# prstrive/SCGaussian

Hardware: AMD Instinct MI355X
Metric: train_iters_per_sec (higher is better)
Workload: dtype f32; 1 GPU; S2: 200000 Gaussians, 1008x756, SH degree 3, fwd+bwd per view (BASELINE configs[1] shape: LLFF-fern 3-view training, 200 k Gaussians @ 1008x756); gaussians=200000, width=1008, height=756, sh_degree=3, visible=174771, views=3, parallelism=single, ranks_seen=1, launched_by=single process, grad_bucket_bytes=0, grad_bucket_bytes_per_view=0

## Files before the change

### scgaussian_amd/csrc/binning_tiles.hip

```cpp
#include "scg_common.h"
#include "tile_sort.h"
#include "tile_walk.h"

#include <mutex>

namespace scg {

constexpr int kTileBlocksSmall = 128;
constexpr int kTileBlocksLarge = 256;
constexpr int64_t kLargeFrame = 1ll << 20;
constexpr int kLargeScene = 100000;
constexpr int kSortSmallMax = 2048;
constexpr int kSortDenseMax = 4096;
constexpr int kSortMidMax = 8192;
constexpr int kVeryLong = 16384;
constexpr int kSort8Max = 4096;
constexpr int kSortBigLdsMax = 16384;
constexpr int kMaxDynLds = 152 * 1024;

template <class F>
__device__ __forceinline__ void visit_instances(const uint2* __restrict__ rects, int grid_x, uint32_t ga, uint32_t gb,
                                                F&& f) {
    const int lane = lane_id();
    for (uint32_t g0 = ga; g0 < gb; g0 += kWave) {
// ... 115 lines not shown
    return sum;
}

__device__ __forceinline__ uint32_t block_exclusive_256(uint32_t v, uint32_t* s_red, uint32_t& total) {
    const int lane = lane_id(), w = wave_id();
    uint32_t inc = v;
#pragma unroll
    for (int off = 1; off < kWave; off <<= 1) {
        const uint32_t n = (uint32_t)__shfl_up((int)inc, off, kWave);
        if (lane >= off) inc += n;
    }
    __syncthreads();
    if (lane == kWave - 1) s_red[w] = inc;
    __syncthreads();
    uint32_t before = 0;
    total = 0;
#pragma unroll
    for (int k = 0; k < kScatterWaves; ++k) {
        const uint32_t sk = s_red[k];
        if (k < w) before += sk;
        total += sk;
    }
    return before + inc - v;
}

__device__ __forceinline__ void publish_tile_starts(int x, int n_tiles, const uint32_t* __restrict__ tile_total,
                                                    const uint32_t* __restrict__ tile_part,
                                                    uint32_t* __restrict__ tile_start, uint2* __restrict__ ranges,
                                                    uint32_t capacity, uint32_t* __restrict__ class_counts,
                                                    uint32_t* __restrict__ mid_tiles, uint32_t* __restrict__ big_tiles,
                                                    uint32_t small_max, const uint32_t* __restrict__ len_hist,
                                                    const uint8_t* __restrict__ tile_class,
                                                    uint32_t* __restrict__ cost_out, const uint32_t* __restrict__ bcost_in,
                                                    uint8_t* q_class ,
                                                    uint32_t* __restrict__ nr_out) {
    __shared__ uint32_t s_red[kScatterWaves];
    __shared__ uint32_t s_first[kLenClasses];
    __shared__ uint32_t s_cnt[kLenClasses];
    const int per = (n_tiles + 7) >> 3;
    const int t0 = x * per, t1 = min(t0 + per, n_tiles);
    const int lane = lane_id();
    if (threadIdx.x < kLenClasses) {
        uint32_t before = 0;
        for (int k = (int)threadIdx.x + 1; k < kLenClasses; ++k) before += len_hist[x * kLenClasses + k];
        s_first[threadIdx.x] = before;
        s_cnt[threadIdx.x] = 0u;
    }
    uint32_t carry = totals_before(tile_total, tile_part, min(t0, n_tiles), s_red);
    uint32_t* order = reinterpret_cast<uint32_t*>(ranges) + 2 * (size_t)n_tiles;
    for (int k0 = t0; k0 < t1; k0 += kScatterThreads) {
        const int t = k0 + (int)threadIdx.x;
        const bool in = t < t1;
        const uint32_t cnt = in ? tile_total[t] : 0u;
        uint32_t total;
        const uint32_t run = carry + block_exclusive_256(cnt, s_red, total);
        carry += total;
        uint32_t len = 0;
        if (in) {
            tile_start[t] = run;
            const uint32_t lo = min(run, capacity), hi = min(run + cnt, capacity);
            ranges[t] = (hi > lo) ? make_uint2(lo, hi) : make_uint2(0u, 0u);
            len = hi - lo;
            if (t == n_tiles - 1) {
                tile_start[n_tiles] = run + cnt;
                if (nr_out) *nr_out = run + cnt;
            }
            if (cost_out) cost_out[t] = 0u;
            const int c = (int)tile_class[t];
            order[t0 + s_first[c] + atomicAdd(&s_cnt[c], 1u)] = (uint32_t)t;
        }
        const bool is_big = len > (uint32_t)kSortMidMax, is_mid = !is_big && len > small_max;
        const uint64_t m_mid = __ballot(is_mid), m_big = __ballot(is_big);
        const uint64_t m_split = __ballot(len > (uint32_t)kVeryLong);
        if (lane == 0 && m_split) atomicAdd(&class_counts[3], (uint32_t)__popcll(m_split));
        uint32_t base_mid = 0, base_big = 0;
        if (lane == 0) {
            if (m_mid) base_mid = atomicAdd(&class_counts[0], (uint32_t)__popcll(m_mid));
            if (m_big) base_big = atomicAdd(&class_counts[1], (uint32_t)__popcll(m_big));
        }
        base_mid = (uint32_t)__shfl((int)base_mid, 0, kWave);
        base_big = (uint32_t)__shfl((int)base_big, 0, kWave);
        const uint64_t below = (lane == 0) ? 0ull : (~0ull >> (kWave - lane));
        if (is_mid) mid_tiles[base_mid + (uint32_t)__popcll(m_mid & below)] = (uint32_t)t;
        if (is_big) big_tiles[base_big + (uint32_t)__popcll(m_big & below)] = (uint32_t)t;
    }
    for (int k = max(t0, t1) + (int)threadIdx.x; k < t0 + per; k += kScatterThreads) order[k] = (uint32_t)n_tiles;

    uint32_t* order_q = order + (size_t)tile_order_slots(n_tiles);
    const int slots8 = tile_order_slots(n_tiles) >> 3;
    const int nq = 4 * max(t1 - t0, 0);
    __syncthreads();
    if (!bcost_in) {
        for (int e = threadIdx.x; e < 4 * slots8; e += kScatterThreads) {
            const uint32_t t = order[t0 + (e >> 2)];
            order_q[4 * (size_t)t0 + e] = (t < (uint32_t)n_tiles) ? 4u * t + (uint32_t)(e & 3) : 4u * (uint32_t)n_tiles;
        }
        return;
    }
    auto qclass = [&](int e) {
        const uint32_t c = bcost_in[4 * (size_t)t0 + e];
        const int k = (int)(__float_as_uint((float)c) >> 19) - ((127 + 4) << 4);
        return max(0, min(kLenClasses - 1, k));
    };
    if (threadIdx.x < kLenClasses) s_cnt[threadIdx.x] = 0u;
    __syncthreads();
    for (int e = threadIdx.x; e < nq; e += kScatterThreads) {
        const int c = qclass(e);
        q_class[e] = (uint8_t)c;
        atomicAdd(&s_cnt[c], 1u);
    }
    __syncthreads();
    if (threadIdx.x < kLenClasses) {
        uint32_t before = 0;
        for (int k = (int)threadIdx.x + 1; k < kLenClasses; ++k) before += s_cnt[k];
        s_first[threadIdx.x] = before;
    }
    __syncthreads();
    if (threadIdx.x < kLenClasses) s_cnt[threadIdx.x] = 0u;
    __syncthreads();
    for (int e = threadIdx.x; e < nq; e += kScatterThreads) {
        const int c = (int)q_class[e];
        order_q[4 * (size_t)t0 + s_first[c] + atomicAdd(&s_cnt[c], 1u)] = 4u * (uint32_t)t0 + (uint32_t)e;
    }
    for (int e = nq + (int)threadIdx.x; e < 4 * slots8; e += kScatterThreads) order_q[4 * (size_t)t0 + e] = 4u * (uint32_t)n_tiles;
}

__device__ __forceinline__ void band_rows(int gy, int band, int& r0, int& r1) {
    r0 = (int)((int64_t)gy * band / kBands);
    r1 = (int)((int64_t)gy * (band + 1) / kBands);
}

__global__ __launch_bounds__(kScatterThreads) void tile_scatter_kernel(const uint2* __restrict__ rects, uint32_t P,
                                                                   int grid_x, int grid_y, int n_slices,
                                                                   const uint32_t* __restrict__ table,
                                                                   const uint32_t* __restrict__ tile_total,
                                                                   const uint32_t* __restrict__ tile_part,
                                                                   uint32_t* __restrict__ point_list,
                                                                   uint32_t capacity,
                                                                   uint32_t* __restrict__ tile_start,
                                                                   uint2* __restrict__ ranges,
                                                                   uint32_t* __restrict__ class_counts,
                                                                   uint32_t* __restrict__ mid_tiles,
                                                                   uint32_t* __restrict__ big_tiles, uint32_t small_max,
                                                                   const uint32_t* __restrict__ len_hist,
                                                                   const uint8_t* __restrict__ tile_class,
                                                                   uint32_t* __restrict__ cost_out, int block_slices,
                                                                   const uint32_t* __restrict__ bcost_in,
                                                                   uint32_t* __restrict__ nr_out) {
    extern __shared__ __attribute__((aligned(16))) unsigned char smem[];
    uint32_t* cursor = reinterpret_cast<uint32_t*>(smem);
    __shared__ uint2 s_qrect[kScatterWaves][kQueue];
    __shared__ uint32_t s_qid[kScatterWaves][kQueue];
    __shared__ uint32_t s_red[2 * kScatterWaves];
    const int n_tiles = grid_x * grid_y;
    if (blockIdx.x < kBands) {
        publish_tile_starts((int)blockIdx.x, n_tiles, tile_total, tile_part, tile_start, ranges, capacity, class_counts,
                            mid_tiles, big_tiles, small_max, len_hist, tile_class, cost_out, bcost_in,
                            smem ,
                            nr_out);
        return;
    }
#ifdef SCG_PROBE_TIMELINE
    uint32_t* tl = cost_out ? cost_out + n_tiles + ((size_t)blockIdx.x * kScatterWaves + wave_id()) * 8 : nullptr;
    const uint32_t tl0 = (uint32_t)wall_clock64();
    uint32_t tl_walk = 0, tl_nwalk = 0, tl_most = 0;
#endif
    const int wg = (int)blockIdx.x - kBands;
    const int band = wg & (kBands - 1), slice = wg >> 3;
    int r0, r1;
    band_rows(grid_y, band, r0, r1);
    const int t_lo = r0 * grid_x, nt = (r1 - r0) * grid_x;
    if (nt == 0) return;
    const int w = wave_id(), lane = lane_id();
    uint32_t sa, sb, dummy;
    if (block_slices) {
        block_slice(P, (uint32_t)n_slices, (uint32_t)slice, sa, sb);
        sa = min(sa * (uint32_t)kBlock, P);
        sb = min(sb * (uint32_t)kBlock, P);
    } else {
        wave_slice(P, (uint32_t)n_slices, (uint32_t)slice, 0u, sa, dummy);
        wave_slice(P, (uint32_t)n_slices, (uint32_t)slice, (uint32_t)kBinWaves - 1u, dummy, sb);
    }
    const uint32_t ga = sa + (uint32_t)((uint64_t)(sb - sa) * w / kScatterWaves);
    const uint32_t gb = sa + (uint32_t)((uint64_t)(sb - sa) * (w + 1) / kScatterWaves);
    constexpr int kAhead = 2;
    auto fetch = [&](uint32_t g) { return (g < gb) ? rects[g] : make_uint2(0u, 0u); };
    uint2 r_q[kAhead];
#pragma unroll
    for (int a = 0; a < kAhead; ++a) r_q[a] = fetch(ga + (uint32_t)(a * kWave + lane));
    const uint32_t* row = table + (size_t)slice * n_tiles + t_lo;
    constexpr int kRowRegs = 8;
    uint32_t row_pre[kRowRegs];
#pragma unroll
    for (int j = 0; j < kRowRegs; ++j) {
        const int k = j * kScatterThreads + (int)threadIdx.x;
        row_pre[j] = (k < nt) ? row[k] : 0u;
    }
    {
        const int full = t_lo / kColTiles;
        uint32_t before = 0;
        const int tail_k = full * kColTiles + (int)threadIdx.x;
        const uint32_t part0 = tile_part[min((int)threadIdx.x, max(full - 1, 0))];
        const uint32_t tail0 = tile_total[min(tail_k, n_tiles - 1)];
        uint32_t tot_pre[kRowRegs];
#pragma unroll
        for (int j = 0; j < kRowRegs; ++j) tot_pre[j] = tile_total[t_lo + min(j * kScatterThreads + (int)threadIdx.x, nt - 1)];
#pragma unroll
        for (int j = 0; j < kRowRegs; ++j) {
            const int k = j * kScatterThreads + (int)threadIdx.x;
            if (k < nt) cursor[k] = tot_pre[j];
        }
        for (int k = kRowRegs * kScatterThreads + (int)threadIdx.x; k < nt; k += kScatterThreads) cursor[k] = tile_total[t_lo + k];
        if ((int)threadIdx.x < full) before += part0;
        if (tail_k < t_lo) before += tail0;
        for (int k = (int)threadIdx.x + kScatterThreads; k < full; k += kScatterThreads) before += tile_part[k];
#pragma unroll
        for (int off = 32; off > 0; off >>= 1) before += (uint32_t)__shfl_xor((int)before, off, kWave);
        __syncthreads();
        const int share = (nt + kScatterThreads - 1) / kScatterThreads;
        const int k_a = min((int)threadIdx.x * share, nt), k_b = min(k_a + share, nt);
        uint32_t mine = 0;
        for (int k = k_a; k < k_b; ++k) mine += cursor[k];
        uint32_t inc = mine;
#pragma unroll
        for (int off = 1; off < kWave; off <<= 1) {
            const uint32_t n = (uint32_t)__shfl_up((int)inc, off, kWave);
            if (lane >= off) inc += n;
        }
        if (lane == kWave - 1) { s_red[w] = inc; s_red[kScatterWaves + w] = before; }
        __syncthreads();
        uint32_t start = inc - mine;
#pragma unroll
        for (int k = 0; k < kScatterWaves; ++k) start += s_red[kScatterWaves + k] + (k < w ? s_red[k] : 0u);
        for (int k = k_a; k < k_b; ++k) {
            const uint32_t cnt = cursor[k];
            cursor[k] = start;
            start += cnt;
        }
        __syncthreads();
#pragma unroll
        for (int j = 0; j < kRowRegs; ++j) {
            const int k = j * kScatterThreads + (int)threadIdx.x;
            if (k < nt) cursor[k] += row_pre[j];
        }
        for (int k = kRowRegs * kScatterThreads + (int)threadIdx.x; k < nt; k += kScatterThreads) cursor[k] += row[k];
        if (threadIdx.x < kWave) cursor[nt + threadIdx.x] = 0u;
    }
    __syncthreads();

#ifdef SCG_PROBE_TIMELINE
    const uint32_t tl1 = (uint32_t)wall_clock64();
#endif
    uint2* qrect = s_qrect[w];
    uint32_t* qid = s_qid[w];
    auto drop = [&](uint32_t tile, uint32_t id) {
        const uint32_t pos = atomicAdd(&cursor[tile - (uint32_t)t_lo], 1u);
        if (pos < capacity) point_list[pos] = id;
    };
    auto scatter_rects = [&](uint2 r, uint32_t g) {
#ifdef SCG_PROBE_TIMELINE
        const uint32_t tw0 = (uint32_t)wall_clock64();
#endif
        const uint32_t wd = r.y & 0xFFFFu, ht = r.y >> 16;
        const uint32_t cnt = wd * ht;
        const uint32_t dump = (uint32_t)nt + (uint32_t)lane;
        uint32_t small = (cnt <= kCoopThreshold) ? cnt : 0u;
        uint32_t x = 0, row_tile = (r.x >> 16) * (uint32_t)grid_x + (r.x & 0xFFFFu) - (uint32_t)t_lo;
        uint32_t most = small;
#pragma unroll
        for (int off = 32; off > 0; off >>= 1) most = max(most, (uint32_t)__shfl_xor((int)most, off, kWave));
        for (uint32_t k = 0; k < most; k += 4) {
            uint32_t slot[4], pos[4];
#pragma unroll
            for (int u = 0; u < 4; ++u) {
                slot[u] = (k + u < small) ? row_tile + x : dump;
                if (++x == wd) { x = 0; row_tile += (uint32_t)grid_x; }
            }
#pragma unroll
            for (int u = 0; u < 4; ++u) pos[u] = atomicAdd(&cursor[slot[u]], 1u);
#pragma unroll
            for (int u = 0; u < 4; ++u)
                if (k + u < small && pos[u] < capacity) point_list[pos[u]] = g;
        }
        walk_rects(cnt > kCoopThreshold ? r : make_uint2(0u, 0u), g, grid_x, drop);
#ifdef SCG_PROBE_TIMELINE
        tl_walk += (uint32_t)wall_clock64() - tw0; tl_nwalk += 1; tl_most += most;
#endif
    };
    int qn = 0;
    for (uint32_t g0 = ga; g0 < gb; g0 += kWave) {
        const uint32_t g = g0 + lane;
        const uint2 r = r_q[0];
#pragma unroll
        for (int a = 0; a + 1 < kAhead; ++a) r_q[a] = r_q[a + 1];
        r_q[kAhead - 1] = fetch(g + kAhead * kWave);
        const int y0 = max((int)(r.x >> 16), r0), y1 = min((int)(r.x >> 16) + (int)(r.y >> 16), r1);
        const bool touches = (r.y & 0xFFFFu) != 0u && y1 > y0;
        const uint64_t m = __ballot(touches);
        if (touches) {
            const int at = qn + (int)__builtin_amdgcn_mbcnt_hi((uint32_t)(m >> 32), __builtin_amdgcn_mbcnt_lo((uint32_t)m, 0u));
            qrect[at] = make_uint2((r.x & 0xFFFFu) | ((uint32_t)y0 << 16), (r.y & 0xFFFFu) | ((uint32_t)(y1 - y0) << 16));
            qid[at] = g;
        }
        qn += __popcll(m);
        __builtin_amdgcn_fence(__ATOMIC_ACQ_REL, "wavefront");
        __builtin_amdgcn_wave_barrier();
        if (qn >= kWave) {
            const uint2 qr = qrect[lane];
            const uint32_t qg = qid[lane];
            const uint2 mr = qrect[kWave + lane];
            const uint32_t mg = qid[kWave + lane];
            __builtin_amdgcn_fence(__ATOMIC_ACQ_REL, "wavefront");
            __builtin_amdgcn_wave_barrier();
            qn -= kWave;
            if (lane < qn) { qrect[lane] = mr; qid[lane] = mg; }
            __builtin_amdgcn_fence(__ATOMIC_ACQ_REL, "wavefront");
            __builtin_amdgcn_wave_barrier();
            scatter_rects(qr, qg);
        }
    }
    if (qn > 0) {
        uint2 qr = make_uint2(0u, 0u);
        uint32_t qg = 0;
        if (lane < qn) { qr = qrect[lane]; qg = qid[lane]; }
        scatter_rects(qr, qg);
    }
#ifdef SCG_PROBE_TIMELINE
    if (tl && lane == 0) {
        tl[0] = tl0; tl[1] = tl1; tl[2] = (uint32_t)wall_clock64(); tl[3] = tl_walk; tl[4] = tl_nwalk; tl[5] = tl_most;
        tl[6] = gb - ga; tl[7] = 0xC0FFEEu;
    }
#endif
}

__device__ __forceinline__ void sort_tile_in_lds(uint64_t* s_keys, const uint32_t* __restrict__ depth_keys,
                                                 uint32_t* __restrict__ list, int n) {
    for (int i = threadIdx.x; i < n; i += (int)blockDim.x) {
        const uint32_t id = list[i];
        s_keys[i] = ((uint64_t)depth_keys[id] << 32) | (uint64_t)id;
    }
    __syncthreads();
    bitonic_sort_asc(s_keys, n, false);
    __syncthreads();
    for (int i = threadIdx.x; i < n; i += (int)blockDim.x) list[i] = (uint32_t)s_keys[i];
}

template <int NW, int MAX_N>
__global__ __launch_bounds__(NW * kWave) void tile_sort_kernel(const uint2* __restrict__ ranges,
                                                               const uint32_t* __restrict__ depth_keys,
                                                               uint32_t* __restrict__ point_list, int id_bits) {
    __shared__ TileSortLds<NW, MAX_N> L;
    const uint2 r = ranges[blockIdx.x];
    const int n = (int)(r.y - r.x);
    if (n < 2 || n > MAX_N) return;
    sort_one_tile<NW, MAX_N, MAX_N>(L, r, depth_keys, point_list, id_bits);
}

constexpr int kRareThreads = 16 * kWave;
constexpr int kLongBuckets = 8192;

__device__ __forceinline__ void sort_big_tile(unsigned char* smem, const uint2 r, const uint32_t* __restrict__ depth_keys,
                                              uint32_t* __restrict__ point_list, uint64_t* __restrict__ spill,
                                              uint64_t* __restrict__ spill2) {
    const int n = (int)(r.y - r.x);
    uint32_t* list = point_list + r.x;
    uint64_t* keys = spill + r.x;
    if (!sort_long_list<kRareThreads, kLongBuckets>(smem, depth_keys, list, n, keys, spill2 + r.x)) {
        __syncthreads();
        if (n <= kSortBigLdsMax) {
            sort_tile_in_lds(reinterpret_cast<uint64_t*>(smem), depth_keys, list, n);
        } else {
            for (int i = threadIdx.x; i < n; i += kRareThreads) {
                const uint32_t id = list[i];
                keys[i] = ((uint64_t)depth_keys[id] << 32) | (uint64_t)id;
            }
            __syncthreads();
            bitonic_sort_asc(keys, n, true);
            __syncthreads();
            for (int i = threadIdx.x; i < n; i += kRareThreads) list[i] = (uint32_t)keys[i];
        }
    }
}

constexpr int kSegTarget = 1024;
constexpr int kSplitBatch = 16;
constexpr int kSegMaxPerTile = 8192;
static_assert(kSegTarget + kLongBucketMax <= kSort8Max, "a segment must fit the 8-wave sort");
static_assert(kLongBucketMax <= kSegTarget, "consecutive bucket starts must be at most a segment apart: no segment index is skipped");

__device__ __forceinline__ bool split_long_list(unsigned char* smem, const uint2 r, const uint32_t* __restrict__ depth_keys,
                                                uint32_t* __restrict__ point_list, uint64_t* __restrict__ A,
                                                uint32_t* __restrict__ seg_count, uint2* __restrict__ segments) {
    constexpr int T = kRareThreads, NW = T / kWave, PER = kLongBuckets / T;
    uint32_t* cnt = reinterpret_cast<uint32_t*>(smem);
    uint32_t* cur = cnt + kLongBuckets + 4;
    uint32_t* red = cur + kLongBuckets;
    uint32_t* pm = red + 2 * NW + 4;
    const int n = (int)(r.y - r.x);
    uint32_t* list = point_list + r.x;
    const int t = threadIdx.x, w = wave_id(), lane = lane_id();
    const int n_seg = (n + kSegTarget - 1) / kSegTarget;
    if (n_seg > kSegMaxPerTile) return false;
    uint32_t kmin, kmax;
    {
        const uint32_t key = depth_keys[list[(int)(((int64_t)t * n) / T)]];
        kmin = key; kmax = key;
    }
    for (int b = t; b < kLongBuckets; b += T) cnt[b] = 0u;
    for (int m = t; m <= n_seg; m += T) pm[m] = (uint32_t)n;
#pragma unroll
    for (int off = 32; off > 0; off >>= 1) {
        kmin = min(kmin, (uint32_t)__shfl_xor((int)kmin, off, kWave));
        kmax = max(kmax, (uint32_t)__shfl_xor((int)kmax, off, kWave));
    }
    if (lane == 0) { red[2 * w] = kmin; red[2 * w + 1] = kmax; }
    __syncthreads();
#pragma unroll
    for (int k = 0; k < NW; ++k) { kmin = min(kmin, red[2 * k]); kmax = max(kmax, red[2 * k + 1]); }
    const int sh = __builtin_clz((kmax - kmin) | 1u);
    auto bucket_of = [&](uint64_t comp) {
        const uint32_t key = (uint32_t)(comp >> 32);
        return __umulhi((min(max(key, kmin), kmax) - kmin) << sh, (uint32_t)kLongBuckets);
    };
    for (int i0 = t; i0 < n; i0 += kSplitBatch * T) {
        uint32_t id[kSplitBatch], key[kSplitBatch];
#pragma unroll
        for (int u = 0; u < kSplitBatch; ++u) id[u] = list[min(i0 + u * T, n - 1)];
#pragma unroll
        for (int u = 0; u < kSplitBatch; ++u) key[u] = depth_keys[id[u]];
#pragma unroll
        for (int u = 0; u < kSplitBatch; ++u) {
            if (i0 + u * T < n) {
                const uint64_t comp = ((uint64_t)key[u] << 32) | (uint64_t)id[u];
                A[i0 + u * T] = comp;
                atomicAdd(&cnt[bucket_of(comp)], 1u);
            }
        }
    }
    __syncthreads();
// ... 341 lines not shown
```

### scgaussian_amd/csrc/geometry.hip

```cpp
#include "scg_common.h"
#include "tile_walk.h"

#include <type_traits>

#pragma clang fp contract(off)

namespace scg {

__constant__ const float kC0 = 0.28209479177387814f;
__constant__ const float kC1 = 0.4886025119029199f;
__constant__ const float kC2[5] = {1.0925484305920792f, -1.0925484305920792f, 0.31539156525252005f,
                                   -1.0925484305920792f, 0.5462742152960396f};
__constant__ const float kC3[7] = {-0.5900435899266435f, 2.890611442640554f, -0.4570457994644658f,
                                   0.3731763325901154f, -0.4570457994644658f, 1.445305721320277f,
                                   -0.5900435899266435f};

struct Mat16 { float m[16]; };

__device__ __forceinline__ Mat16 load16(const float* __restrict__ p) {
    Mat16 r;
#pragma unroll
    for (int i = 0; i < 16; ++i) r.m[i] = p[i];
    return r;
}
// ... 314 lines not shown
        const float lam1 = mid + sqrtf(fmaxf(mid * mid - p.det, 0.1f));
        const float radius_f = ceilf(3.0f * sqrtf(lam1));
        const float ndc_x = p.hx * p.m_w;
        const float ndc_y = p.hy * p.m_w;
        px = ((ndc_x + 1.0f) * (float)f.W - 1.0f) * 0.5f;
        py = ((ndc_y + 1.0f) * (float)f.H - 1.0f) * 0.5f;
        int minx, miny, maxx, maxy;
        tile_rect(px, py, radius_f, f.gx, f.gy, minx, miny, maxx, maxy);
        const int tiles = (maxx - minx) * (maxy - miny);
        ok = tiles > 0;
        if (ok) {
            my_tiles = (uint32_t)tiles;
            radius_i = (int)fminf(fmaxf(radius_f, 0.0f), 2.0e9f);
            rect = make_uint2((uint32_t)minx | ((uint32_t)miny << 16),
                              (uint32_t)(maxx - minx) | ((uint32_t)(maxy - miny) << 16));
            tz = p.tz;
        }
    }
    constexpr bool has_colors = DEG < 0;
    constexpr int K = has_colors ? 1 : (DEG + 1) * (DEG + 1);
    float sh[(3 * K + 3) / 4 * 4];
#ifdef SCG_PROBE_TIMELINE
    { float pin = con_a; asm volatile("" : "+v"(pin)); }
    const uint32_t tp_math = (uint32_t)wall_clock64();
#endif
    if (!has_colors) src.template load_sh<K>(ok ? i : 0, sh);
    between(rect);
#ifdef SCG_PROBE_TIMELINE
    const uint32_t tp_between = (uint32_t)wall_clock64();
    asm volatile("" : "+v"(sh[0]), "+v"(sh[(3 * K + 3) / 4 * 4 - 1]));
    const uint32_t tp_sh = (uint32_t)wall_clock64();
    g_tp[0] += tp_math - g_tp[4]; g_tp[1] += tp_between - tp_math; g_tp[2] += tp_sh - tp_between; g_tp[4] = tp_sh;
#endif
    if (ok) {
        float rgb[3];
        if (has_colors) {
            rgb[0] = in.rgb[0]; rgb[1] = in.rgb[1]; rgb[2] = in.rgb[2];
        } else {
            float dx = in.x - f.campos[0], dy = in.y - f.campos[1], dz = in.z - f.campos[2];
            const float len = sqrtf(dx * dx + dy * dy + dz * dz);
            dx = dx / len; dy = dy / len; dz = dz / len;
            eval_sh<(DEG < 0 ? 0 : DEG)>(sh, dx, dy, dz, rgb);
#pragma unroll
            for (int c = 0; c < 3; ++c) {
                rgb[c] = rgb[c] + 0.5f;
                if (rgb[c] < 0.0f) { clamp_bits |= (uint8_t)(1u << c); rgb[c] = 0.0f; }
            }
        }
        sa = make_float4(px, py, con_a, con_b);
        const float opa = in.opacity;
        sb = make_float4(con_c, opa, 2.0f * logf(255.0f * opa) * 1.001f + 0.01f, -con_b / con_c);
        sc = make_float4(rgb[0], rgb[1], rgb[2], tz);
    }
    const int lane = lane_id();
    stage[3 * lane + 0] = sa;
    stage[3 * lane + 1] = sb;
    stage[3 * lane + 2] = sc;
    reinterpret_cast<uint4*>(stage + 3 * kWave)[lane] = make_uint4((uint32_t)radius_i, (uint32_t)clamp_bits, rect.x, rect.y);
    return my_tiles;
}

template <int DEG, class Src>
__device__ __forceinline__ void geometry_forward_body(
    const FrameDev& f, const Src& src, float4* __restrict__ splats,
    int32_t* __restrict__ radii, uint8_t* __restrict__ clamped, uint2* __restrict__ rects,
    uint32_t* __restrict__ depth_keys, uint32_t* __restrict__ block_sums) {
    __shared__ uint32_t s_wave_sum[kBlock / kWave];
    __shared__ float4 s_stage[(kBlock / kWave) * kStageVec];
    const int i = blockIdx.x * kBlock + threadIdx.x;
    const bool valid = i < f.P;
    const GeoIn in = src.template load<(DEG < 0)>(valid ? i : f.P - 1);
    const Mat16 V = load16(f.view);
    const Mat16 PM = load16(f.proj);
    float4* stage = s_stage + kStageVec * wave_id();
#ifdef SCG_PROBE_TIMELINE
    uint32_t tp_dummy[5] = {0u, 0u, 0u, 0u, 0u};
#endif
    const uint32_t my_tiles = geometry_forward_one<DEG>(f, V, PM, i, valid, in, src, stage,
                                                        [](uint2) {}
#ifdef SCG_PROBE_TIMELINE
                                                        , tp_dummy
#endif
                                                        );
    flush_stage(stage, i - lane_id(), f.P, splats, radii, clamped, rects, depth_keys);

    uint32_t s = my_tiles;
#pragma unroll
    for (int off = 32; off > 0; off >>= 1) s += __shfl_down(s, off, kWave);
    if (lane_id() == 0) s_wave_sum[wave_id()] = s;
    __syncthreads();
    if (threadIdx.x == 0) block_sums[blockIdx.x] = s_wave_sum[0] + s_wave_sum[1] + s_wave_sum[2] + s_wave_sum[3];
}

template <int DEG>
__global__ __launch_bounds__(kBlock) void geometry_forward_kernel(
    FrameDev f, const float* __restrict__ means3D, const float* __restrict__ opacities,
    const float* __restrict__ shs, const float* __restrict__ colors_precomp, const float* __restrict__ scales,
    const float* __restrict__ rotations, const float* __restrict__ cov3D_precomp, float4* __restrict__ splats,
    int32_t* __restrict__ radii, uint8_t* __restrict__ clamped, uint2* __restrict__ rects,
    uint32_t* __restrict__ depth_keys, uint32_t* __restrict__ block_sums, int sh_vec16) {
    const TensorSource src{means3D, opacities, shs, colors_precomp, scales, rotations, cov3D_precomp, f.M, sh_vec16};
    geometry_forward_body<DEG>(f, src, splats, radii, clamped, rects, depth_keys, block_sums);
}

template <int DEG>
__global__ __launch_bounds__(kBlock) void geometry_forward_model_kernel(
    FrameDev f, ScgModel model, float4* __restrict__ splats, int32_t* __restrict__ radii, uint8_t* __restrict__ clamped,
    uint2* __restrict__ rects, uint32_t* __restrict__ depth_keys, uint32_t* __restrict__ block_sums) {
    const ModelSource src{model};
    geometry_forward_body<DEG>(f, src, splats, radii, clamped, rects, depth_keys, block_sums);
}

__host__ __device__ __forceinline__ size_t geometry_hist_stage_offset(int n_tiles, int max_blocks) {
    return ((size_t)(n_tiles + max_blocks) * sizeof(uint32_t) + 15) & ~(size_t)15;
}
__host__ __device__ __forceinline__ size_t geometry_hist_lds_bytes(int n_tiles, int max_blocks) {
    return geometry_hist_stage_offset(n_tiles, max_blocks) + (size_t)(kBinThreads / kWave) * kStageVec * sizeof(float4);
}

template <int DEG, class Src>
__device__ __forceinline__ void geometry_hist_body(
    const FrameDev& f, const Src& src, float4* __restrict__ splats,
    int32_t* __restrict__ radii, uint8_t* __restrict__ clamped, uint2* __restrict__ rects,
    uint32_t* __restrict__ depth_keys, uint32_t* __restrict__ block_sums,
    uint32_t* __restrict__ table, uint32_t* __restrict__ class_counts, uint32_t* __restrict__ len_hist, int max_blocks) {
    extern __shared__ __attribute__((aligned(16))) unsigned char smem[];
    uint32_t* hist = reinterpret_cast<uint32_t*>(smem);
    const int n_tiles = f.gx * f.gy;
    uint32_t* s_blk = hist + n_tiles;
    float4* stage = reinterpret_cast<float4*>(smem + geometry_hist_stage_offset(n_tiles, max_blocks)) + kStageVec * wave_id();
    uint32_t blk_a, blk_b;
    block_slice((uint32_t)f.P, gridDim.x, blockIdx.x, blk_a, blk_b);
    const int lane = lane_id();
    uint32_t chunk = 4u * blk_a + (uint32_t)wave_id();
    auto fetch = [&](uint32_t c) {
        const int g = (int)(c * kWave) + lane;
        return src.template load<(DEG < 0)>(min(g, f.P - 1));
    };
    const Mat16 V = load16(f.view);
    const Mat16 PM = load16(f.proj);
    if (blockIdx.x == 0) {
        if (threadIdx.x < 4) class_counts[threadIdx.x] = 0u;
        len_hist[threadIdx.x] = 0u;
    }
    for (int t = threadIdx.x; t < n_tiles + max_blocks; t += kBinThreads) hist[t] = 0;
    uint32_t* next_chunk = s_blk + (max_blocks - 1);
    __syncthreads();
    if (threadIdx.x == 0) *next_chunk = 4u * blk_a + (uint32_t)kBinWaves;
    __syncthreads();
    int pending = -1;
#ifdef SCG_PROBE_TIMELINE
    uint32_t g_tp[5] = {0u, 0u, 0u, 0u, (uint32_t)wall_clock64()};
    const uint32_t tp_begin = g_tp[4];
    uint32_t tp_iters = 0;
#endif
    while (chunk < 4u * blk_b) {
        const int i = (int)(chunk * kWave) + lane;
        const GeoIn in = fetch(chunk);
        uint32_t grabbed = 0;
        if (lane == 0) grabbed = atomicAdd(next_chunk, 1u);
        const uint32_t my_tiles = geometry_forward_one<DEG>(
            f, V, PM, i, i < f.P, in, src, stage, [&](uint2 rect) {
                if (pending >= 0) flush_stage(stage, pending, f.P, splats, radii, clamped, rects, depth_keys);
                walk_rects(rect, (uint32_t)i, f.gx, [&](uint32_t tile, uint32_t) { atomicAdd(&hist[tile], 1u); });
            }
#ifdef SCG_PROBE_TIMELINE
            , g_tp
#endif
            );
#ifdef SCG_PROBE_TIMELINE
        { const uint32_t t = (uint32_t)wall_clock64(); g_tp[3] += t - g_tp[4]; g_tp[4] = t; ++tp_iters; }
#endif
        pending = i - lane;
        uint32_t s = my_tiles;
#pragma unroll
        for (int off = 32; off > 0; off >>= 1) s += __shfl_down(s, off, kWave);
        if (lane == 0 && s) atomicAdd(&s_blk[(chunk >> 2) - blk_a], s);
        chunk = (uint32_t)__builtin_amdgcn_readfirstlane((int)grabbed);
    }
    if (pending >= 0) flush_stage(stage, pending, f.P, splats, radii, clamped, rects, depth_keys);
#ifdef SCG_PROBE_TIMELINE
    const uint32_t tp_loop_end = (uint32_t)wall_clock64();
#endif
    __syncthreads();
#ifdef SCG_PROBE_TIMELINE
    if (f.cost_out && lane == 0) {
        uint32_t* tl = f.cost_out + n_tiles + 65792 + ((size_t)blockIdx.x * kBinWaves + wave_id()) * 8;
        tl[0] = tp_begin; tl[1] = g_tp[0]; tl[2] = g_tp[1]; tl[3] = g_tp[2]; tl[4] = g_tp[3]; tl[5] = tp_loop_end;
        tl[6] = (uint32_t)wall_clock64(); tl[7] = 0xC0FFEE00u | tp_iters;
    }
#endif
    uint32_t* row = table + (size_t)blockIdx.x * n_tiles;
    for (int t = threadIdx.x; t < n_tiles; t += kBinThreads) row[t] = hist[t];
    for (uint32_t k = threadIdx.x; k < blk_b - blk_a; k += kBinThreads) block_sums[blk_a + k] = s_blk[k];
}

template <int DEG>
__global__ __launch_bounds__(kBinThreads) void geometry_hist_kernel(
    FrameDev f, const float* __restrict__ means3D, const float* __restrict__ opacities,
    const float* __restrict__ shs, const float* __restrict__ colors_precomp, const float* __restrict__ scales,
    const float* __restrict__ rotations, const float* __restrict__ cov3D_precomp, float4* __restrict__ splats,
    int32_t* __restrict__ radii, uint8_t* __restrict__ clamped, uint2* __restrict__ rects,
    uint32_t* __restrict__ depth_keys, uint32_t* __restrict__ block_sums, int sh_vec16,
    uint32_t* __restrict__ table, uint32_t* __restrict__ class_counts, uint32_t* __restrict__ len_hist, int max_blocks) {
    const TensorSource src{means3D, opacities, shs, colors_precomp, scales, rotations, cov3D_precomp, f.M, sh_vec16};
    geometry_hist_body<DEG>(f, src, splats, radii, clamped, rects, depth_keys, block_sums, table, class_counts, len_hist, max_blocks);
}

template <int DEG>
__global__ __launch_bounds__(kBinThreads) void geometry_hist_model_kernel(
    FrameDev f, ScgModel model, float4* __restrict__ splats, int32_t* __restrict__ radii, uint8_t* __restrict__ clamped,
    uint2* __restrict__ rects, uint32_t* __restrict__ depth_keys, uint32_t* __restrict__ block_sums,
    uint32_t* __restrict__ table, uint32_t* __restrict__ class_counts, uint32_t* __restrict__ len_hist, int max_blocks) {
    const ModelSource src{model};
    geometry_hist_body<DEG>(f, src, splats, radii, clamped, rects, depth_keys, block_sums, table, class_counts, len_hist, max_blocks);
}

template <int DEG>
__device__ __forceinline__ void sh_basis_grads(float x, float y, float z, float* basis, float* bx, float* by, float* bz) {
    basis[0] = kC0; bx[0] = by[0] = bz[0] = 0.f;
    if (DEG > 0) {
        basis[1] = -kC1 * y; bx[1] = 0.f; by[1] = -kC1; bz[1] = 0.f;
        basis[2] = kC1 * z;  bx[2] = 0.f; by[2] = 0.f; bz[2] = kC1;
        basis[3] = -kC1 * x; bx[3] = -kC1; by[3] = 0.f; bz[3] = 0.f;
    }
    if (DEG > 1) {
        const float xx = x * x, yy = y * y, zz = z * z, xy = x * y, yz = y * z, xz = x * z;
        basis[4] = kC2[0] * xy;                    bx[4] = kC2[0] * y; by[4] = kC2[0] * x; bz[4] = 0.f;
        basis[5] = kC2[1] * yz;                    bx[5] = 0.f; by[5] = kC2[1] * z; bz[5] = kC2[1] * y;
        basis[6] = kC2[2] * (2.0f * zz - xx - yy); bx[6] = kC2[2] * -2.0f * x; by[6] = kC2[2] * -2.0f * y; bz[6] = kC2[2] * 4.0f * z;
        basis[7] = kC2[3] * xz;                    bx[7] = kC2[3] * z; by[7] = 0.f; bz[7] = kC2[3] * x;
        basis[8] = kC2[4] * (xx - yy);             bx[8] = kC2[4] * 2.0f * x; by[8] = kC2[4] * -2.0f * y; bz[8] = 0.f;
        if (DEG > 2) {
            basis[9] = kC3[0] * y * (3.0f * xx - yy);
            bx[9] = kC3[0] * 6.0f * xy; by[9] = kC3[0] * (3.0f * xx - 3.0f * yy); bz[9] = 0.f;
            basis[10] = kC3[1] * xy * z;
            bx[10] = kC3[1] * yz; by[10] = kC3[1] * xz; bz[10] = kC3[1] * xy;
            basis[11] = kC3[2] * y * (4.0f * zz - xx - yy);
            bx[11] = kC3[2] * -2.0f * xy; by[11] = kC3[2] * (4.0f * zz - xx - 3.0f * yy); bz[11] = kC3[2] * 8.0f * yz;
            basis[12] = kC3[3] * z * (2.0f * zz - 3.0f * xx - 3.0f * yy);
            bx[12] = kC3[3] * -6.0f * xz; by[12] = kC3[3] * -6.0f * yz; bz[12] = kC3[3] * (6.0f * zz - 3.0f * xx - 3.0f * yy);
            basis[13] = kC3[4] * x * (4.0f * zz - xx - yy);
            bx[13] = kC3[4] * (4.0f * zz - 3.0f * xx - yy); by[13] = kC3[4] * -2.0f * xy; bz[13] = kC3[4] * 8.0f * xz;
            basis[14] = kC3[5] * z * (xx - yy);
            bx[14] = kC3[5] * 2.0f * xz; by[14] = kC3[5] * -2.0f * yz; bz[14] = kC3[5] * (xx - yy);
            basis[15] = kC3[6] * x * (xx - 3.0f * yy);
            bx[15] = kC3[6] * (3.0f * xx - 3.0f * yy); by[15] = kC3[6] * -6.0f * xy; bz[15] = 0.f;
        }
    }
}

template <int DEG, bool STREAM = false>
__device__ __forceinline__ void sh_backward(const float* rec, bool vec16, float x, float y, float z,
                                            const float* dRGB, float* dsh_rec, int M,
                                            float& ddx, float& ddy, float& ddz, bool acc,
                                            int sw = -1) {
    auto at = [&](int j) { return sw < 0 ? j : ((((j >> 2) ^ sw) << 2) | (j & 3)); };
    constexpr int K = (DEG + 1) * (DEG + 1);
    float sh[STREAM ? 3 : (3 * K + 3) / 4 * 4];
    if (!STREAM) load_sh<K>(rec, vec16, sh);
    float basis[K];
    float bx[K], by[K], bz[K];
    sh_basis_grads<DEG>(x, y, z, basis, bx, by, bz);
    ddx = ddy = ddz = 0.f;
#pragma unroll
    for (int k = 0; k < K; ++k) {
        float s0, s1, s2;
        if (STREAM) { s0 = rec[at(3 * k)]; s1 = rec[at(3 * k + 1)]; s2 = rec[at(3 * k + 2)]; }
        else { s0 = sh[3 * k]; s1 = sh[3 * k + 1]; s2 = sh[3 * k + 2]; }
        const float g = s0 * dRGB[0] + s1 * dRGB[1] + s2 * dRGB[2];
        ddx += g * bx[k]; ddy += g * by[k]; ddz += g * bz[k];
        if (acc) {
            dsh_rec[at(3 * k + 0)] += basis[k] * dRGB[0];
            dsh_rec[at(3 * k + 1)] += basis[k] * dRGB[1];
            dsh_rec[at(3 * k + 2)] += basis[k] * dRGB[2];
        } else {
            dsh_rec[at(3 * k + 0)] = basis[k] * dRGB[0];
            dsh_rec[at(3 * k + 1)] = basis[k] * dRGB[1];
            dsh_rec[at(3 * k + 2)] = basis[k] * dRGB[2];
        }
    }
    if (!acc)
        for (int k = 3 * K; k < 3 * M; ++k) dsh_rec[at(k)] = 0.f;
}

__device__ __forceinline__ void geometry_backward_one(const FrameDev& f, const Mat16& V, const Mat16& PM, const GeoIn& in,
                                                      bool has_cov, float4& ga, float4& gb, float* dm, float* dm2, float& d_op,
                                                      float* ds, float* dq, float* dcov) {
    const float x = in.x, y = in.y, z = in.z;
    const float opac = in.opacity;
    d_op = (opac > 0.0f) ? ga.w / opac : 0.0f;

    Proj p;
    project(f, V, PM, x, y, z, p);
    if (has_cov) {
#pragma unroll
        for (int k = 0; k < 6; ++k) p.cov[k] = in.a[k];
    } else {
        cov3d_from_scale_rot(in, f.mod, p);
    }
    cov2d(f, V, p);
    {
        const float con_a = p.C * p.det_inv, con_b = -p.B * p.det_inv, con_c = p.A * p.det_inv;
        const float sx = ga.x, sy = ga.y;
        ga.x = -(con_a * sx + con_b * sy);
        ga.y = -(con_b * sx + con_c * sy);
        gb.x *= -0.5f; gb.y = -gb.y; gb.z *= -0.5f;
    }

    const float di2 = p.det_inv * p.det_inv;
    const float dA = di2 * (-p.C * p.C * gb.x + p.B * p.C * gb.y - p.B * p.B * gb.z);
    const float dC = di2 * (-p.B * p.B * gb.x + p.A * p.B * gb.y - p.A * p.A * gb.z);
    const float dB = di2 * (2.0f * p.B * p.C * gb.x - (p.A * p.C + p.B * p.B) * gb.y + 2.0f * p.A * p.B * gb.z);

    const float T0[3] = {p.T00, p.T01, p.T02};
    const float T1[3] = {p.T10, p.T11, p.T12};
    float Ms[9];
#pragma unroll
    for (int j = 0; j < 3; ++j)
#pragma unroll
        for (int k = 0; k < 3; ++k)
            Ms[3 * j + k] = dA * T0[j] * T0[k] + 0.5f * dB * (T0[j] * T1[k] + T1[j] * T0[k]) + dC * T1[j] * T1[k];
    const float u[3] = {p.u0, p.u1, p.u2};
    const float v[3] = {p.v0, p.v1, p.v2};
    float dT0[3], dT1[3];
#pragma unroll
    for (int k = 0; k < 3; ++k) {
        dT0[k] = 2.0f * dA * u[k] + dB * v[k];
        dT1[k] = dB * u[k] + 2.0f * dC * v[k];
    }
    const float dJ00 = dT0[0] * V.m[0] + dT0[1] * V.m[4] + dT0[2] * V.m[8];
    const float dJ02 = dT0[0] * V.m[2] + dT0[1] * V.m[6] + dT0[2] * V.m[10];
    const float dJ11 = dT1[0] * V.m[1] + dT1[1] * V.m[5] + dT1[2] * V.m[9];
    const float dJ12 = dT1[0] * V.m[2] + dT1[1] * V.m[6] + dT1[2] * V.m[10];
    const float itz = 1.0f / p.tz;
    const float itz2 = itz * itz;
    const float itz3 = itz2 * itz;
    const float dtx = p.cl_x ? 0.f : -f.focal_x * itz2 * dJ02;
    const float dty = p.cl_y ? 0.f : -f.focal_y * itz2 * dJ12;
    float dtz = -f.focal_x * itz2 * dJ00 - f.focal_y * itz2 * dJ11 +
                2.0f * f.focal_x * p.t_x * itz3 * dJ02 + 2.0f * f.focal_y * p.t_y * itz3 * dJ12;
    dtz += ga.z;
// ... 623 lines not shown
```

### scgaussian_amd/csrc/tile_walk.h

```cpp
#pragma once

#include "scg_common.h"

namespace scg {

constexpr uint32_t kCoopThreshold = 48;

__device__ __forceinline__ void divmod_small(uint32_t n, uint32_t d, uint32_t& q, uint32_t& r) {
    q = (uint32_t)((float)n * __builtin_amdgcn_rcpf((float)d));
    int rem = (int)n - (int)(q * d);
    if (rem < 0) { q -= 1; rem += (int)d; }
    if (rem >= (int)d) { q += 1; rem -= (int)d; }
    r = (uint32_t)rem;
}

template <class F>
__device__ __forceinline__ void walk_rects(uint2 r, uint32_t g, int grid_x, F&& f) {
    const int lane = lane_id();
    const uint32_t wd = r.y & 0xFFFFu, ht = r.y >> 16;
    const uint32_t cnt = wd * ht;
    if (cnt && cnt <= kCoopThreshold) {
        uint32_t row_tile = (r.x >> 16) * (uint32_t)grid_x + (r.x & 0xFFFFu);
        for (uint32_t y = 0; y < ht; ++y, row_tile += (uint32_t)grid_x)
            for (uint32_t x = 0; x < wd; ++x) f(row_tile + x, g);
    }
    uint64_t big = __ballot(cnt > kCoopThreshold);
    while (big) {
        const int l = __builtin_ctzll(big);
        big &= big - 1;
        const uint32_t bx = (uint32_t)__shfl((int)r.x, l, kWave);
        const uint32_t by = (uint32_t)__shfl((int)r.y, l, kWave);
        const uint32_t bg = (uint32_t)__shfl((int)g, l, kWave);
        const uint32_t bw = by & 0xFFFFu, bn = bw * (by >> 16);
        const uint32_t org = (bx >> 16) * (uint32_t)grid_x + (bx & 0xFFFFu);
        for (uint32_t k = lane; k < bn; k += kWave) {
            uint32_t qy, qx;
            divmod_small(k, bw, qy, qx);
            f(org + qy * (uint32_t)grid_x + qx, bg);
        }
    }
}

constexpr int kBinThreads = 1024;
constexpr int kBinWaves = kBinThreads / kWave;

__device__ __forceinline__ void wave_slice(uint32_t P, uint32_t nblocks, uint32_t b, uint32_t w, uint32_t& ga,
                                           uint32_t& gb) {
    const uint64_t slots = (uint64_t)nblocks * kBinWaves;
    const uint64_t s = (uint64_t)b * kBinWaves + w;
    ga = (uint32_t)(s * P / slots);
    gb = (uint32_t)((s + 1) * P / slots);
}

__host__ __device__ __forceinline__ void block_slice(uint32_t P, uint32_t nblocks, uint32_t b, uint32_t& blk_a, uint32_t& blk_b) {
    const uint64_t nb256 = ((uint64_t)P + kBlock - 1) / kBlock;
    blk_a = (uint32_t)((uint64_t)b * nb256 / nblocks);
    blk_b = (uint32_t)((uint64_t)(b + 1) * nb256 / nblocks);
}

}
```

Measured before the change: 4326 iters/s.

## Load-balance tile scatter across wave via prefix-sum instance distribution

Replaces the per-lane small-rect loop plus cooperative big-rect walk in the binning scatter with a wave-wide load-balanced walk. Each lane's tile count is prefix-summed with DPP, segment heads are marked in LDS, and every lane then handles consecutive instances in rounds of four, recovering the owning Gaussian with ballot and shuffle. This targets divergence where one lane's large rect stalls the wave, at the cost of extra shuffles, LDS mark traffic and divmod per instance. Probe-only trip counting is added to the geometry histogram timeline.

```diff
diff --git a/scgaussian_amd/csrc/binning_tiles.hip b/scgaussian_amd/csrc/binning_tiles.hip
--- a/scgaussian_amd/csrc/binning_tiles.hip
+++ b/scgaussian_amd/csrc/binning_tiles.hip
@@ -291,6 +291,7 @@
     __shared__ uint2 s_qrect[kScatterWaves][kQueue];
     __shared__ uint32_t s_qid[kScatterWaves][kQueue];
     __shared__ uint32_t s_red[2 * kScatterWaves];
+    __shared__ __attribute__((aligned(4))) uint8_t s_marks[kScatterWaves][kWalkMarks];
     const int n_tiles = grid_x * grid_y;
     if (blockIdx.x < kBands) {
         publish_tile_starts((int)blockIdx.x, n_tiles, tile_total, tile_part, tile_start, ranges, capacity, class_counts,
@@ -392,38 +393,32 @@
 #endif
     uint2* qrect = s_qrect[w];
     uint32_t* qid = s_qid[w];
-    auto drop = [&](uint32_t tile, uint32_t id) {
-        const uint32_t pos = atomicAdd(&cursor[tile - (uint32_t)t_lo], 1u);
-        if (pos < capacity) point_list[pos] = id;
-    };
+    uint8_t* marks = s_marks[w];
     auto scatter_rects = [&](uint2 r, uint32_t g) {
 #ifdef SCG_PROBE_TIMELINE
         const uint32_t tw0 = (uint32_t)wall_clock64();
 #endif
-        const uint32_t wd = r.y & 0xFFFFu, ht = r.y >> 16;
-        const uint32_t cnt = wd * ht;
         const uint32_t dump = (uint32_t)nt + (uint32_t)lane;
-        uint32_t small = (cnt <= kCoopThreshold) ? cnt : 0u;
-        uint32_t x = 0, row_tile = (r.x >> 16) * (uint32_t)grid_x + (r.x & 0xFFFFu) - (uint32_t)t_lo;
-        uint32_t most = small;
-#pragma unroll
-        for (int off = 32; off > 0; off >>= 1) most = max(most, (uint32_t)__shfl_xor((int)most, off, kWave));
-        for (uint32_t k = 0; k < most; k += 4) {
-            uint32_t slot[4], pos[4];
-#pragma unroll
-            for (int u = 0; u < 4; ++u) {
-                slot[u] = (k + u < small) ? row_tile + x : dump;
-                if (++x == wd) { x = 0; row_tile += (uint32_t)grid_x; }
-            }
-#pragma unroll
-            for (int u = 0; u < 4; ++u) pos[u] = atomicAdd(&cursor[slot[u]], 1u);
-#pragma unroll
-            for (int u = 0; u < 4; ++u)
-                if (k + u < small && pos[u] < capacity) point_list[pos[u]] = g;
-        }
-        walk_rects(cnt > kCoopThreshold ? r : make_uint2(0u, 0u), g, grid_x, drop);
+        uint32_t slot[kWalkRounds], id[kWalkRounds];
+        const uint32_t n_inst = walk_instances(
+            r, g, grid_x, marks,
+            [&](auto u, bool valid, uint32_t tile, uint32_t gid) {
+                slot[decltype(u)::value] = valid ? tile - (uint32_t)t_lo : dump;
+                id[decltype(u)::value] = gid;
+            },
+            [&](auto n_rounds) {
+                constexpr int NR = decltype(n_rounds)::value;
+                uint32_t pos[NR];
+#pragma unroll
+                for (int u = 0; u < NR; ++u) pos[u] = atomicAdd(&cursor[slot[u]], 1u);
+#pragma unroll
+                for (int u = 0; u < NR; ++u)
+                    if (slot[u] != dump && pos[u] < capacity) point_list[pos[u]] = id[u];
+            });
 #ifdef SCG_PROBE_TIMELINE
-        tl_walk += (uint32_t)wall_clock64() - tw0; tl_nwalk += 1; tl_most += most;
+        tl_walk += (uint32_t)wall_clock64() - tw0; tl_nwalk += 1; tl_most += (n_inst + kWave - 1) / kWave;
+#else
+        (void)n_inst;
 #endif
     };
     int qn = 0;
diff --git a/scgaussian_amd/csrc/geometry.hip b/scgaussian_amd/csrc/geometry.hip
--- a/scgaussian_amd/csrc/geometry.hip
+++ b/scgaussian_amd/csrc/geometry.hip
@@ -490,7 +490,7 @@
 #ifdef SCG_PROBE_TIMELINE
     uint32_t g_tp[5] = {0u, 0u, 0u, 0u, (uint32_t)wall_clock64()};
     const uint32_t tp_begin = g_tp[4];
-    uint32_t tp_iters = 0;
+    uint32_t tp_iters = 0, tp_trips = 0;
 #endif
     while (chunk < 4u * blk_b) {
         const int i = (int)(chunk * kWave) + lane;
@@ -501,6 +501,17 @@
             f, V, PM, i, i < f.P, in, src, stage, [&](uint2 rect) {
                 if (pending >= 0) flush_stage(stage, pending, f.P, splats, radii, clamped, rects, depth_keys);
                 walk_rects(rect, (uint32_t)i, f.gx, [&](uint32_t tile, uint32_t) { atomicAdd(&hist[tile], 1u); });
+#ifdef SCG_PROBE_TIMELINE
+                {
+                    const uint32_t c = (rect.y & 0xFFFFu) * (rect.y >> 16);
+                    uint32_t most = c <= kCoopThreshold ? c : 0u, coop = c > kCoopThreshold ? (c + 63u) / 64u : 0u;
+                    for (int off = 32; off > 0; off >>= 1) {
+                        most = max(most, (uint32_t)__shfl_xor((int)most, off, kWave));
+                        coop += (uint32_t)__shfl_xor((int)coop, off, kWave);
+                    }
+                    tp_trips += most + coop;
+                }
+#endif
             }
 #ifdef SCG_PROBE_TIMELINE
             , g_tp
@@ -525,7 +536,7 @@
     if (f.cost_out && lane == 0) {
         uint32_t* tl = f.cost_out + n_tiles + 65792 + ((size_t)blockIdx.x * kBinWaves + wave_id()) * 8;
         tl[0] = tp_begin; tl[1] = g_tp[0]; tl[2] = g_tp[1]; tl[3] = g_tp[2]; tl[4] = g_tp[3]; tl[5] = tp_loop_end;
-        tl[6] = (uint32_t)wall_clock64(); tl[7] = 0xC0FFEE00u | tp_iters;
+        tl[6] = (uint32_t)wall_clock64(); tl[7] = 0xC7000000u | (min(tp_trips, 0xFFFFu) << 8) | min(tp_iters, 0xFFu);
     }
 #endif
     uint32_t* row = table + (size_t)blockIdx.x * n_tiles;
diff --git a/scgaussian_amd/csrc/tile_walk.h b/scgaussian_amd/csrc/tile_walk.h
--- a/scgaussian_amd/csrc/tile_walk.h
+++ b/scgaussian_amd/csrc/tile_walk.h
@@ -2,9 +2,10 @@
 
 #include "scg_common.h"
 
+#include <type_traits>
+#include <utility>
+
 namespace scg {
-
-constexpr uint32_t kCoopThreshold = 48;
 
 __device__ __forceinline__ void divmod_small(uint32_t n, uint32_t d, uint32_t& q, uint32_t& r) {
     q = (uint32_t)((float)n * __builtin_amdgcn_rcpf((float)d));
@@ -13,6 +14,8 @@
     if (rem >= (int)d) { q += 1; rem -= (int)d; }
     r = (uint32_t)rem;
 }
+
+constexpr uint32_t kCoopThreshold = 48;
 
 template <class F>
 __device__ __forceinline__ void walk_rects(uint2 r, uint32_t g, int grid_x, F&& f) {
@@ -41,6 +44,98 @@
     }
 }
 
+constexpr int kWalkRounds = 4;
+constexpr int kWalkMarks = kWalkRounds * kWave;
+constexpr uint32_t kNoMark = 0xFFu;
+
+__device__ __forceinline__ void wave_lds_sync() {
+    __builtin_amdgcn_fence(__ATOMIC_ACQ_REL, "wavefront");
+    __builtin_amdgcn_wave_barrier();
+}
+
+__device__ __forceinline__ uint32_t wave_inclusive_sum(uint32_t v) {
+    v += (uint32_t)__builtin_amdgcn_update_dpp(0, (int)v, 0x111, 0xF, 0xF, false);
+    v += (uint32_t)__builtin_amdgcn_update_dpp(0, (int)v, 0x112, 0xF, 0xF, false);
+    v += (uint32_t)__builtin_amdgcn_update_dpp(0, (int)v, 0x114, 0xF, 0xF, false);
+    v += (uint32_t)__builtin_amdgcn_update_dpp(0, (int)v, 0x118, 0xF, 0xF, false);
+    v += (uint32_t)__builtin_amdgcn_update_dpp(0, (int)v, 0x142, 0xA, 0xF, false);
+    v += (uint32_t)__builtin_amdgcn_update_dpp(0, (int)v, 0x143, 0xC, 0xF, false);
+    return v;
+}
+
+template <int... I, class F>
+__device__ __forceinline__ void static_rounds(std::integer_sequence<int, I...>, F&& f) {
+    (f(std::integral_constant<int, I>{}), ...);
+}
+
+template <class Visit, class GroupEnd>
+__device__ __forceinline__ uint32_t walk_instances(uint2 r, uint32_t g, int grid_x, uint8_t* marks, Visit&& visit,
+                                                   GroupEnd&& group_end) {
+    const int lane = lane_id();
+    const uint32_t cnt = (r.y & 0xFFFFu) * (r.y >> 16);
+    const uint32_t incl = wave_inclusive_sum(cnt);
+    const uint32_t first = incl - cnt;
+    const uint32_t total = (uint32_t)__builtin_amdgcn_readlane((int)incl, kWave - 1);
+    const uint32_t le_lo = lane < 32 ? (2u << lane) - 1u : ~0u;
+    const uint32_t le_hi = lane < 32 ? 0u : (2u << (lane - 32)) - 1u;
+
+    auto group = [&](uint32_t base, auto n_rounds) {
+        constexpr int NR = decltype(n_rounds)::value;
+        uint32_t m[NR];
+#pragma unroll
+        for (int u = 0; u < NR; ++u) m[u] = marks[u * kWave + lane];
+        int carry = 0;
+        int owner[NR];
+        bool marked[NR];
+        int carried[NR];
+#pragma unroll
+        for (int u = 0; u < NR; ++u) {
+            const uint64_t heads = __ballot(m[u] != kNoMark);
+            const uint32_t h_lo = (uint32_t)heads & le_lo, h_hi = (uint32_t)(heads >> 32) & le_hi;
+            const int at = h_hi ? 63 - __builtin_clz(h_hi) : 31 - __builtin_clz(h_lo | 1u);
+            owner[u] = __shfl((int)m[u], at, kWave);
+            marked[u] = (h_lo | h_hi) != 0u;
+            carried[u] = carry;
+            if (u + 1 < NR) {
+                const int last = __builtin_amdgcn_readlane((int)m[u], heads ? 63 - __builtin_clzll(heads) : 0);
+                carry = heads ? last : carry;
+            }
+        }
+        uint32_t o_x[NR], o_y[NR], o_first[NR], o_g[NR];
+#pragma unroll
+        for (int u = 0; u < NR; ++u) {
+            const int o = marked[u] ? owner[u] : carried[u];
+            o_x[u] = (uint32_t)__shfl((int)r.x, o, kWave);
+            o_y[u] = (uint32_t)__shfl((int)r.y, o, kWave);
+            o_first[u] = (uint32_t)__shfl((int)first, o, kWave);
+            o_g[u] = (uint32_t)__shfl((int)g, o, kWave);
+        }
+        static_rounds(std::make_integer_sequence<int, NR>{}, [&](auto round) {
+            constexpr int u = decltype(round)::value;
+            const uint32_t k = base + (uint32_t)(u * kWave + lane);
+            uint32_t qy, qx;
+            divmod_small((k - o_first[u]) & 0xFFFFFFu, o_y[u] & 0xFFFFu, qy, qx);
+            uint32_t tile = ((o_x[u] >> 16) + qy) * (uint32_t)grid_x + (o_x[u] & 0xFFFFu) + qx;
+            asm("" : "+v"(tile));
+            visit(round, k < total, tile, o_g[u]);
+        });
+        group_end(n_rounds);
+    };
+    for (uint32_t base = 0; base < total; base += (uint32_t)kWalkMarks) {
+        reinterpret_cast<uint32_t*>(marks)[lane] = 0xFFFFFFFFu;
+        wave_lds_sync();
+        if (cnt && first < base + (uint32_t)kWalkMarks && incl > base) marks[max(first, base) - base] = (uint8_t)lane;
+        wave_lds_sync();
+        const uint32_t left = total - base;
+        if (left > 3u * kWave) group(base, std::integral_constant<int, 4>{});
+        else if (left > 2u * kWave) group(base, std::integral_constant<int, 3>{});
+        else if (left > 1u * kWave) group(base, std::integral_constant<int, 2>{});
+        else group(base, std::integral_constant<int, 1>{});
+        wave_lds_sync();
+    }
+    return total;
+}
+
 constexpr int kBinThreads = 1024;
 constexpr int kBinWaves = kBinThreads / kWave;
 
```

Result: no change. 4308 iters/s (-0.4%).
